# adamjorr/kbbq

Measured on AMD Instinct MI355X. Metric: recalibrated Gbases/sec, higher is better.
Workload: dtype u64

## Files before the change

### kbbq_amd/csrc/engine.hip

```cpp
#include <hip/hip_runtime.h>

#include <algorithm>
#include <cstdarg>
#include <cstdio>
#include <cstdlib>
#include <cstring>
#include <map>
#include <mutex>
#include <string>
#include <thread>
#include <vector>

#include "../../include/kbbq_engine.h"
#include "abi_internal.h"
#include "correct.h"
#include "correct_wave.h"
#include "device_common.h"
#include "host_model.h"

using namespace kbbq;

static thread_local char g_err[512] = "";
int kbbq_fail(int code, const char *fmt, ...) {
    va_list ap;
    va_start(ap, fmt);
    vsnprintf(g_err, sizeof g_err, fmt, ap);
    va_end(ap);
    return code;
}
#define fail kbbq_fail
#define HIP_TRY(expr)                                                                                  \
    do {                                                                                               \
        hipError_t _e = (expr);                                                                        \
        if (_e != hipSuccess)                                                                          \
            return fail(_e == hipErrorOutOfMemory ? KBBQ_ENOMEM : KBBQ_EIO, "%s: %s (%s:%d)", #expr,   \
                        hipGetErrorString(_e), __FILE__, __LINE__);                                    \
    } while (0)

#include "kernels.h"
#include "bucket.h"
#include "long_reads.h"


struct FilterHost {
    FilterSpec spec;
    uint64_t *d_table = nullptr;
    uint64_t *d_patterns = nullptr;
    unsigned long long *d_inserted = nullptr;
    uint64_t table_bytes() const { return spec.n_blocks * kEngineBlockBytes; }
    FiltDev dev() const {
        FiltDev f;
        f.table = reinterpret_cast<ulonglong2 *>(d_table);
        f.patterns = reinterpret_cast<const ulonglong2 *>(d_patterns);
        f.n_blocks = spec.n_blocks;
        const ModMagic mm = make_mod_magic(spec.n_blocks);
        f.mod_magic = mm.m64;
        f.mod_m32 = mm.m32;
        f.salt0 = spec.salt[0];
        f.salt1 = spec.salt[1];
        return f;
    }
};

struct ProfileSlot {
    std::string name;
    uint64_t launches = 0;
    double ms = 0;
};
struct PendingEvent {
    int slot;
    hipEvent_t a, b;
};

struct Options {
    bool no_overlap = false;
    bool no_fastpath = false;
    bool lane_walk = false;
    bool no_pass4_pipeline = false;
    int pass2_side = 2;
    bool tally_general = false;
    bool infer_subset = true;
    bool debug_bucket = false;
    int bucket = -1;
    uint64_t bucket_records = 0;
    uint64_t pass4_piece = 0;
    int scan_blocks = -1;
    int walk_blocks = -1;
    int infer_blocks = 0;
};

struct kbbq_engine {
    kbbq_params p;
    Options opt;
    KParams K;
    hipStream_t stream = nullptr;
    hipStream_t stream2 = nullptr;
    hipEvent_t ev_main = nullptr, ev_side[2] = {nullptr, nullptr};
    hipEvent_t ev_draw = nullptr, ev_ins[2] = {nullptr, nullptr};
    bool ins_pending[2] = {false, false};
    int draw_turn = 0;
    bool side_busy[2] = {false, false};
    bool pass3_shared = false;
    unsigned long long *d_totals = nullptr;
    int side_turn = 0;
    uint32_t *d_qpresent = nullptr;
    uint32_t qpresent[8] = {};
    bool qpresent_known = false;
    uint8_t *d_dq_qslot = nullptr;
    int dq_slots = 0;
    uint32_t *d_rg_present[2] = {nullptr, nullptr};
    hipStream_t cur = nullptr;
    unsigned long long *cur_cnt = nullptr;
    FilterHost filt[2];
    Xoshiro256 seed_state;
    uint64_t draw_threshold = 0;
    bool draw_always = false;
    bool thresholds_set = false;
    std::vector<int32_t> thresholds;
    unsigned long long *d_hist = nullptr;
    uint64_t hist_cycle_words = 0, hist_dinuc_words = 0;
    DqTables dq;
    bool dq_set = false;
    int16_t *d_dq_base = nullptr;
    int8_t *d_dq_cycle = nullptr;
    int8_t *d_dq_dinuc = nullptr;
    void *scratch[24] = {};
    size_t scratch_bytes[24] = {};
    unsigned long long *d_counters = nullptr;
    unsigned int *d_tickets = nullptr;
    struct StageSlot {
        char *dev = nullptr;
        size_t bytes = 0;
        hipEvent_t h2d = nullptr, done[2] = {nullptr, nullptr};
        hipEvent_t d2h = nullptr;
        bool busy[2] = {false, false};
        bool d2h_pending = false;
        uint32_t gen = 0;
    } slot[3];
    int slot_turn = 0, cur_slot = -1;
    bool cur_slot_side = false;
    bool cur_h2d_recorded = false;
    bool async_call = false;
    uint64_t last_ticket = 0;
    hipStream_t copy = nullptr;
    uint64_t stats[4] = {0, 0, 0, 0};
    std::vector<ProfileSlot> prof;
    std::vector<PendingEvent> pending;
    uint32_t *d_qcum = nullptr, *d_errthr = nullptr;
    uint32_t qcum_len = 0;
    struct Buckets {
        int mode[2] = {-1, -1};
        bool allocated = false;
        uint64_t capacity = 0;
        void *l1 = nullptr, *l2 = nullptr;
        uint32_t *l1_cnt = nullptr, *l2_cnt = nullptr, *tickets = nullptr;
        unsigned long long *direct = nullptr;
        bool pending[2] = {false, false};
        double pending_est[2] = {0, 0};
        double frac_trusted = 0.75;
        double frac_used = 0.75;
        uint64_t bases_since[2] = {0, 0}, inserted_at_flush[2] = {0, 0};
        uint64_t flushes[2] = {0, 0};
        hipStream_t stream[2] = {nullptr, nullptr};
        hipEvent_t ev_flush = nullptr;
        unsigned long long *h_inserted = nullptr;
        hipEvent_t ev_est = nullptr;
        bool est_pending = false, est_known = false;
        uint64_t est_bases = 0, est_prev = 0, cur_bases = 0;
    } bk;
    hipEvent_t ev_infer = nullptr, ev_take[2] = {nullptr, nullptr};
    bool take_pending[2] = {false, false};
    int take_turn = 0;
    size_t attr_lds_tally = 0, attr_lds_recal = 0;
    std::map<const void *, size_t> attr_lds_correct;
};

namespace {

int ensure_scratch(kbbq_engine *e, int idx, size_t bytes) {
    if (e->scratch_bytes[idx] >= bytes) return KBBQ_OK;
    if (e->scratch[idx]) {
        HIP_TRY(hipStreamSynchronize(e->stream));
        HIP_TRY(hipStreamSynchronize(e->stream2));
        HIP_TRY(hipFree(e->scratch[idx]));
        e->scratch[idx] = nullptr;
        e->scratch_bytes[idx] = 0;
    }
    const size_t want = bytes + bytes / 8 + 256;
    HIP_TRY(hipMalloc(&e->scratch[idx], want));
    e->scratch_bytes[idx] = want;
    return KBBQ_OK;
}

static void plan_tally_slots(TallyPlan &P, const uint32_t mask[8], int max_slots, int n_rg) {
    memset(P.qslot, 255, sizeof P.qslot);
    memset(P.qof, 0, sizeof P.qof);
    P.n_slots = 0;
    max_slots = std::max(1, std::min(max_slots, 255));
    int top = -1, distinct = 0;
    for (int q = 0; q < KBBQ_NQ; ++q)
        if ((mask[q >> 5] >> (q & 31)) & 1) { top = q; ++distinct; }
    if (top >= 0 && top + 1 <= max_slots && (n_rg <= 1 || 2 * distinct >= top + 1)) {
        for (int q = 0; q <= top; ++q) { P.qof[q] = (uint8_t)q; P.qslot[q] = (uint8_t)q; }
        P.n_slots = top + 1;
        P.identity = 1;
    } else {
        for (int q = 0; q < KBBQ_NQ && P.n_slots < max_slots; ++q)
            if ((mask[q >> 5] >> (q & 31)) & 1) { P.qof[P.n_slots] = (uint8_t)q; P.qslot[q] = (uint8_t)P.n_slots++; }
        P.identity = 0;
    }
    if (P.n_slots == 0) { P.n_slots = 1; P.qof[0] = 0; P.qslot[0] = 0; P.identity = 1; }
    P.rg_base = 0; P.n_rgs = 1; P.cbase = 0; P.direct_cycles = 0;
}

struct Timed {
    kbbq_engine *e;
    int slot = -1;
    hipEvent_t a = nullptr, b = nullptr;
    hipStream_t on = nullptr;
    Timed(kbbq_engine *e_, const char *name, hipStream_t stream = nullptr) : e(e_), on(stream ? stream : e_->stream) {
        if (!(e->p.flags & KBBQ_F_PROFILE)) return;
        for (size_t i = 0; i < e->prof.size(); ++i)
            if (e->prof[i].name == name) slot = (int)i;
        if (slot < 0) {
            ProfileSlot s;
            s.name = name;
            e->prof.push_back(s);
            slot = (int)e->prof.size() - 1;
        }
        hipEventCreate(&a);
        hipEventCreate(&b);
        hipEventRecord(a, on);
    }
    ~Timed() {
        if (slot < 0) return;
        hipEventRecord(b, on);
        PendingEvent pe = {slot, a, b};
        e->pending.push_back(pe);
    }
};

void drain_profile(kbbq_engine *e) {
    for (size_t i = 0; i < e->pending.size(); ++i) {
        PendingEvent &pe = e->pending[i];
        float ms = 0;
        if (hipEventSynchronize(pe.b) == hipSuccess && hipEventElapsedTime(&ms, pe.a, pe.b) == hipSuccess) {
            e->prof[pe.slot].ms += ms;
            e->prof[pe.slot].launches += 1;
        }
        hipEventDestroy(pe.a);
        hipEventDestroy(pe.b);
    }
    e->pending.clear();
}

__global__ void k_add_counters(const unsigned long long *side, const unsigned long long *offcase, unsigned long long *totals) {
// ... 359 lines not shown
        HIP_TRY(hipStreamWaitEvent(e->stream, b.ev_flush, 0));
    }
    if (w == 1 && !barrier) {
        bucket_poll_estimate(e);
        if (!b.est_pending && b.h_inserted) {
            HIP_TRY(hipMemcpyAsync(b.h_inserted, e->filt[1].d_inserted, 8, hipMemcpyDeviceToHost, e->stream));
            HIP_TRY(hipEventRecord(b.ev_est, e->stream));
            b.est_pending = true;
            b.est_bases = b.bases_since[1] + b.cur_bases;
            b.est_prev = b.inserted_at_flush[1];
            if (!b.est_known) {
                HIP_TRY(hipEventSynchronize(b.ev_est));
                bucket_poll_estimate(e);
                b.est_known = true;
            }
        }
    }
    {
        if (e->opt.debug_bucket) fprintf(stderr, "[bucket] flush %d of filter %d: estimate %.3g records over %llu bases (%.4f per base), barrier %d\n",
                           (int)b.flushes[w], w, b.pending_est[w], (unsigned long long)b.bases_since[w], w ? b.frac_trusted : 0.0, (int)barrier);
    }
    b.bases_since[w] = 0;
    b.pending[w] = false;
    b.pending_est[w] = 0;
    b.flushes[w] += 1;
    return KBBQ_OK;
}

int bucket_flush_all(kbbq_engine *e) {
    for (int w = 0; w < 2; ++w) {
        int rc = bucket_flush(e, w);
        if (rc) return rc;
    }
    return KBBQ_OK;
}

int bucket_reserve(kbbq_engine *e, int w, double est, uint64_t bases) {
    kbbq_engine::Buckets &b = e->bk;
    int rc = bucket_flush(e, 1 - w);
    if (rc) return rc;
    b.cur_bases = bases;
    if (b.pending[w] && b.pending_est[w] + est > 0.93 * (double)b.capacity) {
        if ((rc = bucket_flush(e, w, false))) return rc;
        if (w == 1) est = (est - 4096.0) / std::max(1e-9, b.frac_used) * b.frac_trusted + 4096.0;
    }
    b.cur_bases = 0;
    b.pending[w] = true;
    b.pending_est[w] += est;
    b.bases_since[w] += bases;
    return KBBQ_OK;
}

}


extern "C" {

const char *kbbq_last_error(void) { return g_err; }

int kbbq_engine_create(const kbbq_params *params, kbbq_engine **out) {
    if (!params || !out) return fail(KBBQ_EINVAL, "null argument");
    if (params->k < 1 || params->k > KBBQ_MAX_KMER) return fail(KBBQ_ERANGE, "k must be <= %d and > 0", KBBQ_MAX_KMER);
    if (params->n_rg < 1 || params->n_rg > 65535) return fail(KBBQ_EINVAL, "n_rg must be in 1..65535");
    if (params->max_read_len < 1 || params->max_read_len > KBBQ_MAX_READ_LEN)
        return fail(KBBQ_ERANGE, "max_read_len must be in 1..%d", KBBQ_MAX_READ_LEN);
    int ndev = 0;
    if (hipGetDeviceCount(&ndev) != hipSuccess || ndev == 0) return fail(KBBQ_ENODEV, "no HIP device visible");
    if (params->device < 0 || params->device >= ndev) return fail(KBBQ_ENODEV, "device %d of %d", params->device, ndev);
    DeviceGuard create_guard(params->device);
    HIP_TRY(create_guard.err);
    kbbq_engine *e = new kbbq_engine;
    e->p = *params;
    {
        Options &o = e->opt;
        auto env_set = [](const char *name) { const char *v = getenv(name); return v && *v; };
        auto env_int = [](const char *name, int dflt) { const char *v = getenv(name); return v && *v ? atoi(v) : dflt; };
        const int fl = params->flags;
        o.no_overlap = (fl & KBBQ_F_NO_OVERLAP) || env_set("KBBQ_NO_OVERLAP");
        o.no_fastpath = (fl & KBBQ_F_NO_FASTPATH) || env_set("KBBQ_NO_FASTPATH");
        o.lane_walk = (fl & KBBQ_F_LANE_WALK) || (getenv("KBBQ_CORRECT") && !strcmp(getenv("KBBQ_CORRECT"), "lane"));
        o.no_pass4_pipeline = (fl & KBBQ_F_NO_PASS4_PIPELINE) || env_set("KBBQ_NO_PASS4_PIPELINE");
        o.pass2_side = (fl & KBBQ_F_PASS2_INORDER) ? 0 : env_int("KBBQ_PASS2_SIDE", o.pass2_side);
        o.tally_general = env_set("KBBQ_TALLY_GENERAL");
        o.infer_subset = env_int("KBBQ_INFER_SUBSET", 1) != 0;
        o.debug_bucket = env_set("KBBQ_DEBUG_BUCKET");
        o.bucket = (fl & KBBQ_F_BUCKET_ON) ? 1 : (fl & KBBQ_F_BUCKET_OFF) ? 0 : env_set("KBBQ_BUCKET") ? (env_int("KBBQ_BUCKET", 0) != 0 ? 1 : 0) : -1;
        o.bucket_records = env_u64("KBBQ_BUCKET_RECORDS", 0);
        o.pass4_piece = env_u64("KBBQ_PASS4_PIECE", 0);
        o.scan_blocks = env_int("KBBQ_SCAN_BLOCKS", o.scan_blocks);
        o.walk_blocks = env_int("KBBQ_WALK_BLOCKS", o.walk_blocks);
        o.infer_blocks = env_int("KBBQ_INFER_BLOCKS", o.infer_blocks);
    }
    e->K.k = params->k;
    e->K.shift = 2u * (unsigned)(params->k - 1);
    e->K.mask = params->k < 32 ? ((1ULL << (2 * params->k)) - 1) : ~0ULL;
    e->K.nmask_bits = params->k < 32 ? ((1u << params->k) - 1) : 0xFFFFFFFFu;
    const double fprs[2] = {params->fpr_sampled, params->fpr_trusted};
    for (int w = 0; w < 2; ++w) {
        if (!make_filter_spec(params->approx_kmers, fprs[w], params->bloom_seed, e->filt[w].spec)) {
            delete e;
            return fail(KBBQ_EINVAL, "Error: Invalid bloom filter parameters. Adjust parameters and try again.");
        }
    }
    hipError_t he = hipStreamCreateWithFlags(&e->stream, hipStreamNonBlocking);
    if (he == hipSuccess) he = hipStreamCreateWithFlags(&e->stream2, hipStreamNonBlocking);
    if (he == hipSuccess) he = hipEventCreateWithFlags(&e->ev_main, hipEventDisableTiming);
    if (he == hipSuccess) he = hipEventCreateWithFlags(&e->ev_draw, hipEventDisableTiming);
    for (int t = 0; t < 2 && he == hipSuccess; ++t) he = hipEventCreateWithFlags(&e->ev_ins[t], hipEventDisableTiming);
    if (he == hipSuccess) he = hipEventCreateWithFlags(&e->ev_side[0], hipEventDisableTiming);
    if (he == hipSuccess) he = hipEventCreateWithFlags(&e->ev_side[1], hipEventDisableTiming);
    if (he == hipSuccess) he = hipStreamCreateWithFlags(&e->copy, hipStreamNonBlocking);
    if (he == hipSuccess) he = hipEventCreateWithFlags(&e->bk.ev_flush, hipEventDisableTiming);
    if (he == hipSuccess) he = hipEventCreateWithFlags(&e->bk.ev_est, hipEventDisableTiming);
    if (he == hipSuccess) he = hipEventCreateWithFlags(&e->ev_infer, hipEventDisableTiming);
    for (int t = 0; t < 2 && he == hipSuccess; ++t) he = hipEventCreateWithFlags(&e->ev_take[t], hipEventDisableTiming);
    if (he == hipSuccess) he = hipHostMalloc((void **)&e->bk.h_inserted, 64, hipHostMallocDefault);
    for (int i = 0; i < 3 && he == hipSuccess; ++i) {
        he = hipEventCreateWithFlags(&e->slot[i].h2d, hipEventDisableTiming);
        if (he == hipSuccess) he = hipEventCreateWithFlags(&e->slot[i].d2h, hipEventDisableTiming);
        for (int t = 0; t < 2 && he == hipSuccess; ++t) he = hipEventCreateWithFlags(&e->slot[i].done[t], hipEventDisableTiming);
    }
    e->cur = e->stream;
    if (he != hipSuccess) { kbbq_engine_destroy(e); return fail(KBBQ_EIO, "hipStreamCreate: %s", hipGetErrorString(he)); }
#define CREATE_TRY(expr)                                                                           \
    do {                                                                                           \
        hipError_t _e = (expr);                                                                    \
        if (_e != hipSuccess) {                                                                    \
            int code = _e == hipErrorOutOfMemory ? KBBQ_ENOMEM : KBBQ_EIO;                         \
            fail(code, "%s: %s", #expr, hipGetErrorString(_e));                                    \
            kbbq_engine_destroy(e);                                                                \
            return code;                                                                           \
        }                                                                                          \
    } while (0)
    CREATE_TRY(hipMalloc(&e->d_counters, 64));
    CREATE_TRY(hipMemset(e->d_counters, 0, 64));
    CREATE_TRY(hipMalloc(&e->d_tickets, 64));
    CREATE_TRY(hipMemset(e->d_tickets, 0, 64));
    CREATE_TRY(hipMalloc(&e->d_totals, 32));
    CREATE_TRY(hipMemset(e->d_totals, 0, 32));
    e->cur_cnt = e->d_counters;
    CREATE_TRY(hipMalloc(&e->d_dq_qslot, KBBQ_NQ));
    CREATE_TRY(hipMalloc(&e->d_qpresent, 32));
    for (int i = 0; i < 2; ++i) CREATE_TRY(hipMalloc(&e->d_rg_present[i], (((size_t)params->n_rg + 31) / 32) * 4 + 4));
    for (int w = 0; w < 2; ++w) {
        FilterHost &f = e->filt[w];
        CREATE_TRY(hipMalloc(&f.d_table, f.table_bytes()));
        CREATE_TRY(hipMalloc(&f.d_patterns, kNumPatterns * kEngineBlockBytes));
        CREATE_TRY(hipMalloc(&f.d_inserted, 8));
        std::vector<uint64_t> packed(kNumPatterns * 2);
        for (uint64_t i = 0; i < kNumPatterns; ++i) {
            if (!squeeze_block(&f.spec.patterns[i * 8], &packed[i * 2])) {
                kbbq_engine_destroy(e);
                return fail(KBBQ_ESTATE, "pattern %llu uses a bit outside the 128 the generator can reach", (unsigned long long)i);
            }
        }
        CREATE_TRY(hipMemcpy(f.d_patterns, packed.data(), kNumPatterns * kEngineBlockBytes, hipMemcpyHostToDevice));
    }
    e->hist_cycle_words = (uint64_t)params->n_rg * kNQ * 2 * params->max_read_len * 2;
    e->hist_dinuc_words = (uint64_t)params->n_rg * kNQ * 16 * 2;
    CREATE_TRY(hipMalloc(&e->d_hist, (e->hist_cycle_words + e->hist_dinuc_words) * 8));
    CREATE_TRY(hipMalloc(&e->d_dq_base, (size_t)params->n_rg * kNQ * 2));
    CREATE_TRY(hipMalloc(&e->d_dq_cycle, (size_t)params->n_rg * kNQ * 2 * params->max_read_len));
    CREATE_TRY(hipMalloc(&e->d_dq_dinuc, (size_t)params->n_rg * kNQ * 16));
    CREATE_TRY(hipMemcpyToSymbol(HIP_SYMBOL(c_jump), xoshiro_jump_table(), 64 * 4 * 8));
    e->seed_state.seed32(params->seed);
    e->draw_threshold = bernoulli_threshold(params->alpha, &e->draw_always);
// ... 29 lines not shown
        hipFree(e->filt[w].d_inserted);
    }
    hipFree(e->d_hist);
    hipFree(e->d_dq_base);
    hipFree(e->d_dq_cycle);
    hipFree(e->d_dq_dinuc);
    hipFree(e->d_counters);
    hipFree(e->d_tickets);
    hipFree(e->d_totals);
    hipFree(e->d_dq_qslot);
    hipFree(e->d_qpresent);
    hipFree(e->d_rg_present[0]);
    hipFree(e->d_rg_present[1]);
    hipFree(e->d_qcum);
    hipFree(e->d_errthr);
    hipFree(e->bk.l1); hipFree(e->bk.l2); hipFree(e->bk.l1_cnt); hipFree(e->bk.l2_cnt); hipFree(e->bk.tickets); hipFree(e->bk.direct);
    for (int i = 0; i < 24; ++i) hipFree(e->scratch[i]);
    if (e->stream2) { hipStreamSynchronize(e->stream2); hipStreamDestroy(e->stream2); }
    if (e->ev_main) hipEventDestroy(e->ev_main);
    if (e->ev_draw) hipEventDestroy(e->ev_draw);
    for (int t = 0; t < 2; ++t) if (e->ev_ins[t]) hipEventDestroy(e->ev_ins[t]);
    for (int i = 0; i < 2; ++i) if (e->ev_side[i]) hipEventDestroy(e->ev_side[i]);
    if (e->stream) hipStreamDestroy(e->stream);
    delete e;
}

int kbbq_engine_reset(kbbq_engine *e) {
    ENGINE_DEVICE(e);
    if (!e) return fail(KBBQ_EINVAL, "null engine");
    int rc0 = sync_engine(e);
    if (rc0) return rc0;
    for (int w = 0; w < 2; ++w) {
        HIP_TRY(hipMemsetAsync(e->filt[w].d_table, 0, e->filt[w].table_bytes(), e->stream));
        HIP_TRY(hipMemsetAsync(e->filt[w].d_inserted, 0, 8, e->stream));
    }
    HIP_TRY(hipMemsetAsync(e->d_hist, 0, (e->hist_cycle_words + e->hist_dinuc_words) * 8, e->stream));
    HIP_TRY(hipMemsetAsync(e->d_counters, 0, 64, e->stream));
    HIP_TRY(hipMemsetAsync(e->d_totals, 0, 16, e->stream));
    HIP_TRY(hipMemsetAsync(e->d_qpresent, 0, 32, e->stream));
    memset(e->qpresent, 0, sizeof e->qpresent);
    e->qpresent_known = false;
    if (e->bk.allocated) {
        HIP_TRY(hipMemsetAsync(e->bk.l1_cnt, 0, kL1CntBytes, e->stream));
        HIP_TRY(hipMemsetAsync(e->bk.l2_cnt, 0, kL2CntBytes, e->stream));
        HIP_TRY(hipMemsetAsync(e->bk.direct, 0, 8, e->stream));
    }
    e->bk.est_pending = false;
    e->bk.est_known = false;
    e->bk.frac_trusted = 0.75;
    e->bk.stream[0] = e->bk.stream[1] = nullptr;
    for (int w = 0; w < 2; ++w) { e->bk.pending[w] = false; e->bk.pending_est[w] = 0; e->bk.bases_since[w] = 0; e->bk.inserted_at_flush[w] = 0; e->bk.flushes[w] = 0; }
    e->thresholds_set = false;
    e->dq_set = false;
    memset(e->stats, 0, sizeof e->stats);
    return sync_engine(e);
}

int kbbq_engine_sync(kbbq_engine *e) {
    ENGINE_DEVICE(e);
    { int frc = bucket_flush_all(e); if (frc) return frc; }
    if (!e) return fail(KBBQ_EINVAL, "null engine");
    return sync_engine(e);
}

void *kbbq_engine_stream(kbbq_engine *e) { return e ? (void *)e->stream : nullptr; }

int kbbq_engine_dims(kbbq_engine *e, uint64_t *n_rg, uint64_t *n_cycle) {
    if (!e) return fail(KBBQ_EINVAL, "null engine");
    if (n_rg) *n_rg = (uint64_t)e->p.n_rg;
    if (n_cycle) *n_cycle = (uint64_t)e->p.max_read_len;
    return KBBQ_OK;
}

int kbbq_engine_tune(kbbq_engine *e, const char *name, uint64_t value) {
    if (!e || !name) return fail(KBBQ_EINVAL, "null argument");
    if (!strcmp(name, "bucket_records")) {
        if (e->bk.allocated) return fail(KBBQ_ESTATE, "the record buffers are allocated already");
        e->opt.bucket_records = value;
    } else if (!strcmp(name, "pass4_piece")) {
        e->opt.pass4_piece = value;
    } else if (!strcmp(name, "scan_blocks") || !strcmp(name, "walk_blocks") || !strcmp(name, "infer_blocks")) {
        if (value > 17) return fail(KBBQ_EINVAL, "%s: 0 (as many as fit) to 16 workgroups per CU, 17 = default", name);
        (name[0] == 's' ? e->opt.scan_blocks : name[0] == 'w' ? e->opt.walk_blocks : e->opt.infer_blocks) = value == 17 ? (name[0] == 'i' ? 0 : -1) : (int)value;
    } else if (!strcmp(name, "infer_subset")) {
        e->opt.infer_subset = value != 0;
    } else if (!strcmp(name, "pass2_side")) {
        ENGINE_DEVICE(e);
        { int frc = bucket_flush_all(e); if (frc) return frc; }
        int rc = sync_engine(e);
        if (rc) return rc;
        if (value > 2) return fail(KBBQ_EINVAL, "pass2_side: 0, 1 or 2");
        e->opt.pass2_side = (int)value;
        e->bk.stream[0] = e->bk.stream[1] = nullptr;
    } else if (!strcmp(name, "no_overlap")) {
        ENGINE_DEVICE(e);
        { int frc = bucket_flush_all(e); if (frc) return frc; }
        int rc = sync_engine(e);
        if (rc) return rc;
        e->opt.no_overlap = value != 0;
        e->bk.stream[0] = e->bk.stream[1] = nullptr;
    } else {
        return fail(KBBQ_EINVAL, "unknown knob '%s'", name);
    }
    return KBBQ_OK;
}

int kbbq_filter_info_get(kbbq_engine *e, int which, kbbq_filter_info *out) {
    ENGINE_DEVICE(e);
    { int frc = bucket_flush_all(e); if (frc) return frc; }
    if (!e || !out || which < 0 || which > 1) return fail(KBBQ_EINVAL, "bad argument");
    const FilterSpec &s = e->filt[which].spec;
    memset(out, 0, sizeof *out);
    out->bits = s.bits;
    out->bits_unblocked = s.bits_unblocked;
    out->n_blocks = s.n_blocks;
    out->table_bytes = e->filt[which].table_bytes();
    out->random_seed = s.random_seed;
    out->n_hash = s.n_hash;
    out->n_salt = s.n_salt;
    for (uint32_t i = 0; i < s.n_salt; ++i) out->salt[i] = s.salt[i];
    int rc = sync_engine(e);
    if (rc) return rc;
    HIP_TRY(hipMemcpy(&out->inserted, e->filt[which].d_inserted, 8, hipMemcpyDeviceToHost));
    return KBBQ_OK;
}

void *kbbq_filter_device_table(kbbq_engine *e, int which) {
    if (!e || which < 0 || which > 1) return nullptr;
    DeviceGuard guard(e->p.device);
    if (guard.err != hipSuccess || bucket_flush_all(e) != KBBQ_OK) return nullptr;
    return e->filt[which].d_table;
}
void *kbbq_filter_device_counter(kbbq_engine *e, int which) { return e && which >= 0 && which < 2 ? e->filt[which].d_inserted : nullptr; }

int kbbq_filter_download(kbbq_engine *e, int which, uint64_t *host_words, uint64_t n_words) {
    ENGINE_DEVICE(e);
    { int frc = bucket_flush_all(e); if (frc) return frc; }
    if (!e || !host_words || which < 0 || which > 1) return fail(KBBQ_EINVAL, "bad argument");
    const uint64_t n_blocks = e->filt[which].spec.n_blocks;
    if (n_words != n_blocks * 8) return fail(KBBQ_EINVAL, "filter has %llu words", (unsigned long long)n_blocks * 8);
    int rc = sync_engine(e);
    if (rc) return rc;
    const uint64_t chunk = 1 << 20;
    std::vector<uint64_t> packed(chunk * 2);
    for (uint64_t b0 = 0; b0 < n_blocks; b0 += chunk) {
        const uint64_t nb = std::min(chunk, n_blocks - b0);
        HIP_TRY(hipMemcpy(packed.data(), e->filt[which].d_table + b0 * 2, nb * kEngineBlockBytes, hipMemcpyDeviceToHost));
        for (uint64_t b = 0; b < nb; ++b) expand_block(&packed[b * 2], host_words + (b0 + b) * 8);
    }
    return KBBQ_OK;
}

int kbbq_filter_patterns_download(kbbq_engine *e, int which, uint64_t *host_words) {
    ENGINE_DEVICE(e);
    if (!e || !host_words || which < 0 || which > 1) return fail(KBBQ_EINVAL, "bad argument");
    std::vector<uint64_t> packed(kNumPatterns * 2);
    HIP_TRY(hipMemcpy(packed.data(), e->filt[which].d_patterns, kNumPatterns * kEngineBlockBytes, hipMemcpyDeviceToHost));
    for (uint64_t i = 0; i < kNumPatterns; ++i) expand_block(&packed[i * 2], host_words + i * 8);
    return KBBQ_OK;
}

int kbbq_filter_or_from(kbbq_engine *e, int which, const void *src_device, uint64_t word_offset, uint64_t n_words) {
    ENGINE_DEVICE(e);
    { int frc = bucket_flush_all(e); if (frc) return frc; }
    if (!e || !src_device || which < 0 || which > 1) return fail(KBBQ_EINVAL, "bad argument");
    const uint64_t total = e->filt[which].spec.n_blocks * 2;
// ... 773 lines not shown
        raised = lds;
    }
    Timed t(e, "k_correct", e->cur);
    const int blocks = (int)std::min<uint64_t>((R.n_reads + BLOCK - 1) / BLOCK, 256 * 8);
    hipLaunchKernelGGL((k_correct<MAXL, BLOCK>), dim3(blocks), dim3(BLOCK), lds, e->cur, R, e->K, e->filt[1].dev(), list,
                       n_list, tmask, tw, err_bits, patch, e->cur_cnt, 0, (uint32_t *)nullptr);
    HIP_TRY(hipGetLastError());
    return KBBQ_OK;
}

template <int NB, int NN>
static int launch_correct_wave(kbbq_engine *e, ReadsDev R, const uint32_t *list, const uint64_t *tmask, int tw,
                               uint32_t *err_bits, uint32_t *patch) {
    unsigned int *ticket = e->d_tickets + 3 + (e->cur_cnt != e->d_counters ? 1 : 0);
    HIP_TRY(hipMemsetAsync(ticket, 0, 4, e->cur));
    Timed t(e, "k_correct_wave", e->cur);
    const int blocks = wave_grid(R.n_reads, e->pass3_shared ? shared_cap(e, e->opt.walk_blocks, 2, NB <= 5 ? 160 : 512, !R.offsets) : 0);
    hipLaunchKernelGGL((k_correct_wave<NB, NN>), dim3(blocks), dim3(256), 0, e->cur, R, e->K, e->filt[1].dev(), list,
                       (const unsigned long long *)e->cur_cnt, tmask, tw, err_bits, patch, e->cur_cnt, ticket);
    HIP_TRY(hipGetLastError());
    return KBBQ_OK;
}
extern "C" {

static int build_read_index(kbbq_engine *e, const ReadsDev &R, int slot, hipStream_t stream, const uint32_t **index) {
    *index = nullptr;
    if (!R.offsets || !R.n_reads) return KBBQ_OK;
    const size_t entries = R.n_bases / READ_INDEX_STEP + 2;
    int rc = ensure_scratch(e, slot, entries * 4);
    if (rc) return rc;
    hipLaunchKernelGGL(k_read_index, dim3((unsigned)((R.n_reads + 255) / 256)), dim3(256), 0, stream, R.offsets, R.n_reads, (uint32_t *)e->scratch[slot]);
    HIP_TRY(hipGetLastError());
    *index = (const uint32_t *)e->scratch[slot];
    return KBBQ_OK;
}

static int run_tally(kbbq_engine *e, const ReadsDev &R, const uint32_t *err_bits, const uint32_t *patch, int max_len,
                     hipStream_t stream = nullptr) {
    if (!stream) stream = e->cur;
    HistDev H;
    H.cycle = e->d_hist;
    H.dinuc = e->d_hist + e->hist_cycle_words;
    H.n_rg = e->p.n_rg;
    H.n_cycle = e->p.max_read_len;
    const int n_rg = R.rg ? e->p.n_rg : 1;
    const int ccap = std::min(((max_len + 31) / 32) * 32, 192);
    if (!e->qpresent_known) {
        hipLaunchKernelGGL(k_qpresence, dim3(1024), dim3(256), 0, stream, R.qual, R.n_bases, e->d_qpresent);
        HIP_TRY(hipGetLastError());
        HIP_TRY(hipMemcpyAsync(e->qpresent, e->d_qpresent, 32, hipMemcpyDeviceToHost, stream));
        HIP_TRY(hipStreamSynchronize(stream));
    }
    const int n_windows = (max_len + ccap - 1) / ccap;
    const bool direct_cycles = n_windows > kTallyMaxWindows;
    const size_t per_slot = (direct_cycles ? 0 : (size_t)8 * ccap) + 128;
    TallyPlan P;
    plan_tally_slots(P, e->qpresent, (int)((152 * 1024 - 512) / per_slot), n_rg);
    P.direct_cycles = direct_cycles ? 1 : 0;
    const size_t per_rg = (size_t)P.n_slots * per_slot;
    const size_t budget = (size_t)n_rg * per_rg <= 70 * 1024 ? 70 * 1024 : 140 * 1024;
    const int per_launch = (int)std::max<size_t>(1, std::min<size_t>((size_t)n_rg, budget / per_rg));
    const size_t lds = (size_t)per_launch * per_rg + 4 + 256 + 4;
    if (lds > e->attr_lds_tally) {
        HIP_TRY(hipFuncSetAttribute((const void *)k_tally, hipFuncAttributeMaxDynamicSharedMemorySize, (int)lds));
        HIP_TRY(hipFuncSetAttribute((const void *)k_tally_uniform<true>, hipFuncAttributeMaxDynamicSharedMemorySize, (int)lds));
        HIP_TRY(hipFuncSetAttribute((const void *)k_tally_uniform<false>, hipFuncAttributeMaxDynamicSharedMemorySize, (int)lds));
        e->attr_lds_tally = lds;
    }
    const uint64_t groups = (R.n_bases + 15) / 16;
    const int blocks = (int)std::min<uint64_t>((groups + 1023) / 1024, lds <= 76 * 1024 ? 512 : 256);
    const int vec_ok = ((uintptr_t)R.qual & 15) == 0;
    const uint32_t *read_index;
    int rc = build_read_index(e, R, stream == e->stream2 ? 15 : 14, stream, &read_index);
    if (rc) return rc;
    const uint32_t *present = nullptr;
    if (n_rg > per_launch) {
        uint32_t *pr = e->d_rg_present[stream == e->stream2 ? 1 : 0];
        HIP_TRY(hipMemsetAsync(pr, 0, (((size_t)e->p.n_rg + 31) / 32) * 4, stream));
        hipLaunchKernelGGL(k_rg_presence, dim3((unsigned)((R.n_reads + 255) / 256)), dim3(256), 0, stream, R.rg, R.n_reads, (uint32_t)e->p.n_rg, pr);
        present = pr;
    }
    if (!e->opt.tally_general && !R.offsets && n_rg == 1 && n_windows == 1 && R.read_len >= 16 && (int)R.read_len <= ccap && R.n_bases < (1ULL << 32) && vec_ok &&
        e->p.n_rg == 1) {
        const unsigned long long inv_len = ~0ULL / R.read_len + 1;
        Timed t(e, "k_tally", stream);
        if (P.identity) hipLaunchKernelGGL(k_tally_uniform<false>, dim3(blocks), dim3(1024), lds, stream, R, H, err_bits, patch, ccap, 6, inv_len, P);
        else hipLaunchKernelGGL(k_tally_uniform<true>, dim3(blocks), dim3(1024), lds, stream, R, H, err_bits, patch, ccap, 6, inv_len, P);
        HIP_TRY(hipGetLastError());
        return KBBQ_OK;
    }
    Timed t(e, "k_tally", stream);
    for (int g = 0; g < n_rg; g += per_launch)
        for (int w = 0; w < (direct_cycles ? 1 : n_windows); ++w) {
            P.rg_base = g;
            P.n_rgs = std::min(per_launch, n_rg - g);
            P.cbase = w * ccap;
            hipLaunchKernelGGL(k_tally, dim3(blocks), dim3(1024), lds, stream, R, H, err_bits, patch, ccap, 6, vec_ok, P, present, read_index);
        }
    HIP_TRY(hipGetLastError());
    return KBBQ_OK;
}

int kbbq_errors_batch(kbbq_engine *e, const kbbq_reads *reads, uint64_t *errors_out) {
    ENGINE_DEVICE(e);
    { int frc = bucket_flush_all(e); if (frc) return frc; }
    if (!e || !reads) return fail(KBBQ_EINVAL, "null argument");
    const bool own_err = !(errors_out && reads->on_device);
    const bool overlap = own_err && !(errors_out && !reads->on_device) && !e->opt.no_overlap;
    int side = 0, rc;
    if (overlap) {
        side = e->side_turn;
        e->side_turn ^= 1;
        if (e->side_busy[side]) HIP_TRY(hipStreamWaitEvent(e->stream, e->ev_side[side], 0));
    } else {
        if ((rc = sync_engine(e))) return rc;
    }
    e->pass3_shared = overlap;
    HostBatchDone host_done(e, reads);
    ReadsDev R; int max_len;
    if ((rc = device_view(e, reads, &R, &max_len))) return rc;
    const bool long_reads = max_len > kStagedMax;
    const int NW = max_len <= 192 ? 3 : max_len <= 320 ? 5 : !long_reads ? 8 : 8 * ((std::max(1, max_len - e->p.k + 1) + 511) / 512);
    const int s_tmask = side ? 10 : 3, s_dirty = side ? 11 : 4, s_list = side ? 12 : 5, s_err = side ? 8 : 6, s_patch = side ? 9 : 7;
    if ((rc = ensure_scratch(e, s_tmask, R.n_reads * NW * 8))) return rc;
    if ((rc = ensure_scratch(e, s_dirty, R.n_reads))) return rc;
    if ((rc = ensure_scratch(e, s_list, R.n_reads * 4))) return rc;
    if ((rc = ensure_scratch(e, s_patch, R.n_reads * 4))) return rc;
    uint32_t *d_err;
    if (own_err) {
        if ((rc = ensure_scratch(e, s_err, (R.n_bases / 64 + 2) * 8))) return rc;
        d_err = (uint32_t *)e->scratch[s_err];
    } else {
        d_err = (uint32_t *)errors_out;
    }
    e->cur = e->stream;
    e->cur_cnt = e->d_counters + 4 * side;
    struct Restore { kbbq_engine *e; ~Restore() { e->cur = e->stream; e->cur_cnt = e->d_counters; } } restore = {e};
    HIP_TRY(hipMemsetAsync(d_err, 0, (R.n_bases / 64 + 1) * 8, e->cur));
    HIP_TRY(hipMemsetAsync(e->scratch[s_patch], 0, R.n_reads * 4, e->cur));
    HIP_TRY(hipMemsetAsync(e->cur_cnt, 0, 16, e->cur));
    uint64_t *tmask = (uint64_t *)e->scratch[s_tmask];
    uint8_t *dirty = (uint8_t *)e->scratch[s_dirty];
    uint32_t *list = (uint32_t *)e->scratch[s_list];
    uint32_t *patch = (uint32_t *)e->scratch[s_patch];
    const bool no_fast = e->opt.no_fastpath;
    if (long_reads) {
        Timed t(e, "k_scan_trusted_long", e->cur);
        hipLaunchKernelGGL(k_scan_trusted_long, dim3(wave_grid(R.n_reads)), dim3(256), 0, e->cur, R, e->K, e->filt[1].dev(), tmask, NW, dirty);
        HIP_TRY(hipGetLastError());
    } else if ((rc = dispatch_nw<LaunchScan>(max_len, e, R, tmask, dirty, d_err, (!no_fast && e->p.k >= 3) ? 1 : 0, max_len))) return rc;
    {
        Timed t(e, "k_compact", e->cur);
        hipLaunchKernelGGL(k_compact, dim3((unsigned)((R.n_reads + 1023) / 1024)), dim3(1024), 0, e->cur, dirty, R.n_reads, list, e->cur_cnt,
                           long_reads ? 0 : 1);
        HIP_TRY(hipGetLastError());
    }
    if (overlap) {
        HIP_TRY(hipEventRecord(e->ev_main, e->stream));
        HIP_TRY(hipStreamWaitEvent(e->stream2, e->ev_main, 0));
        e->cur = e->stream2;
        e->cur_slot_side = true;
    }
    const bool lane_form = e->opt.lane_walk;
    if (long_reads) {
        rc = launch_correct<0, 64>(e, R, list, e->cur_cnt, tmask, NW, d_err, patch, max_len, side);
    } else if (lane_form || e->p.k < 3) {
// ... 470 lines not shown
```

### kbbq_amd/csrc/kernels.h

```cpp
#pragma once
#include <hip/hip_runtime.h>

#include "../../include/kbbq_engine.h"
#include "correct.h"
#include "correct_wave.h"
#include "device_common.h"

using namespace kbbq;


constexpr int DRAWS_PER_LANE = 4096;

__constant__ uint64_t c_jump[64][4];

__device__ __forceinline__ uint64_t xo_next(uint64_t (&s)[4]) {
    uint64_t x = s[1] * 5;
    x = (x << 7) | (x >> 57);
    x *= 9;
    const uint64_t t = s[1] << 17;
    s[2] ^= s[0];
    s[3] ^= s[1];
    s[1] ^= s[2];
    s[0] ^= s[3];
    s[2] ^= t;
// ... 984 lines not shown
                const int c = (slot % cstep) * 16 + slot / cstep;
                if (c < H.n_cycle) {
                    atomicAdd(&H.cycle[cyc_index(H, 0, q, sec, c) + 1], (unsigned long long)cnt);
                    if (cne) atomicAdd(&H.cycle[cyc_index(H, 0, q, sec, c)], (unsigned long long)cne);
                }
            }
        }
        for (int w = threadIdx.x; w < ns * 16; w += blockDim.x) {
            const uint32_t v = t_di[w], ve = t_die[w];
            const uint64_t cell = (uint64_t)(MAP ? (int)P.qof[w >> 4] : (w >> 4)) * 16 + (w & 15);
            if (v) { t_di[w] = 0; atomicAdd(&H.dinuc[cell * 2 + 1], (unsigned long long)v); }
            if (ve) { t_die[w] = 0; atomicAdd(&H.dinuc[cell * 2], (unsigned long long)ve); }
        }
    };
    const uint64_t n_groups = (R.n_bases + 15) / 16;
    const uint64_t stride = (uint64_t)gridDim.x * blockDim.x;
    const uint64_t iters = (n_groups + stride - 1) / stride;
    const uint64_t flush_every = max((uint64_t)1, (uint64_t)40000 / ((uint64_t)16384 / (uint64_t)L + 2));
    for (uint64_t it = 0; it < iters; ++it) {
        const uint64_t g0 = (it * stride + (uint64_t)blockIdx.x * blockDim.x + threadIdx.x) * 16;
        if (g0 + 16 <= R.n_bases) {
            const uint32_t r = (uint32_t)__umul64hi((unsigned long long)g0, inv_len);
            const int c0 = (int)(g0 - (uint64_t)r * (uint64_t)L);
            const int bpos = L - c0 < 16 ? L - c0 : 16;
            const uint4 qv4 = *reinterpret_cast<const uint4 *>(R.qual + g0);
            uint8_t qv[16];
            memcpy(qv, &qv4, 16);
            const uint32_t bw = (uint32_t)(R.bases[g0 >> 5] >> ((g0 & 31) * 2));
            const uint32_t nw = (uint32_t)(R.nmask[g0 >> 6] >> (g0 & 63)) & 0xFFFFu;
            const uint32_t ew = (err_bits[g0 >> 5] >> (g0 & 31)) & 0xFFFFu;
            int prev_b = 0, prev_n = 1;
            if (g0 > 0) {
                const uint64_t gp = g0 - 1;
                prev_b = (int)((R.bases[gp >> 5] >> ((gp & 31) * 2)) & 3);
                prev_n = (int)((R.nmask[gp >> 6] >> (gp & 63)) & 1);
            }
            const bool two = bpos < 16;
            const bool mine1 = !R.rg || R.rg[r] == 0, mine2 = !two || !R.rg || R.rg[r + 1] == 0;
            const int sec1 = R.flags ? (R.flags[r] & 1) : 0;
            const int sec2 = two && R.flags ? (R.flags[r + 1] & 1) : 0;
            const uint32_t pt1 = patch ? patch[r] : 0u, pt2 = two && patch ? patch[r + 1] : 0u;
            const int pp1 = (pt1 >> 31) ? patch_at(pt1) : -2, pp2 = (pt2 >> 31) ? patch_at(pt2) : -2;
            if (pp1 >= 0 && pp1 == c0 - 1) { prev_b = (int)(pt1 & 3); prev_n = 0; }
#pragma unroll
            for (int i = 0; i < 16; ++i) {
                const bool in2 = i >= bpos;
                const int cyc = c0 + i - (in2 ? L : 0);
                int b = (int)((bw >> (2 * i)) & 3), nn = (int)((nw >> i) & 1);
                if (cyc == (in2 ? pp2 : pp1)) { b = (int)((in2 ? pt2 : pt1) & 3); nn = 0; }
                const int q = qv[i];
                if (in2 ? mine2 : mine1)
                    count(in2 ? sec2 : sec1, q, cyc, (int)((ew >> i) & 1u), cyc >= 1 && q >= minscore && !(nn | prev_n), (prev_b << 2) | b);
                prev_b = b;
                prev_n = nn;
            }
        } else if (g0 < R.n_bases) {
            for (uint64_t g = g0; g < R.n_bases; ++g) {
                const uint64_t r = g / (uint64_t)L;
                const int cyc = (int)(g - r * (uint64_t)L);
                const uint32_t pt = patch ? patch[r] : 0u;
                const int pp = (pt >> 31) ? patch_at(pt) : -2;
                auto base_at = [&](uint64_t x, int cx, int &bb, int &nb) {
                    bb = (int)((R.bases[x >> 5] >> ((x & 31) * 2)) & 3);
                    nb = (int)((R.nmask[x >> 6] >> (x & 63)) & 1);
                    if (cx == pp) { bb = (int)(pt & 3); nb = 0; }
                };
                int b, nn, pb = 0, pn = 1;
                base_at(g, cyc, b, nn);
                if (cyc >= 1) base_at(g - 1, cyc - 1, pb, pn);
                const int q = R.qual[g];
                const int er = (int)((err_bits[g >> 5] >> (g & 31)) & 1u);
                if (!R.rg || R.rg[r] == 0)
                    count(R.flags ? (R.flags[r] & 1) : 0, q, cyc, er, cyc >= 1 && q >= minscore && !(nn | pn), (pb << 2) | b);
            }
        }
        if ((it + 1) % flush_every == 0 || it + 1 == iters) {
            __syncthreads();
            flush();
            __syncthreads();
        }
    }
}

__global__ void __launch_bounds__(256) k_qpresence(const uint8_t *qual, uint64_t n_bases, uint32_t *qpresent) {
    __shared__ uint32_t qseen[8];
    if (threadIdx.x < 8) qseen[threadIdx.x] = 0;
    __syncthreads();
    for (uint64_t i = (uint64_t)blockIdx.x * blockDim.x + threadIdx.x; i < n_bases; i += (uint64_t)gridDim.x * blockDim.x)
        qseen_note(qseen, qual[i]);
    __syncthreads();
    if (threadIdx.x < 8 && qseen[threadIdx.x]) atomicOr(&qpresent[threadIdx.x], qseen[threadIdx.x]);
}

struct DqDev {
    const int16_t *base;
    const int8_t *cycle;
    const int8_t *dinuc;
    const uint8_t *qslot;
    int n_rg, n_cycle, n_slots;
};

__global__ void __launch_bounds__(1024) k_recalibrate(ReadsDev R, DqDev D, uint8_t *out, int minqual, int vec_ok, int lds_rgs,
                                                       const uint32_t *read_index, uint64_t base0, uint64_t base1) {
    extern __shared__ uint8_t l_tab[];
    uint8_t *l_qslot = l_tab;
    const int ns = D.n_slots;
    const int cyc_cells = ns * 2 * D.n_cycle, di_bytes = ns * 16, base_bytes = KBBQ_NQ * 2;
    const int cyc_bytes = 2 * cyc_cells;
    const int per_rg = (cyc_bytes + di_bytes + base_bytes + 3) & ~3;
    uint8_t *l_rg = l_tab + 256;
    if (threadIdx.x < 256) l_qslot[threadIdx.x] = D.qslot[threadIdx.x];
    __syncthreads();
    for (int i = threadIdx.x; i < lds_rgs * KBBQ_NQ; i += blockDim.x) {
        const int rg = i / KBBQ_NQ, q = i % KBBQ_NQ;
        reinterpret_cast<int16_t *>(l_rg + (size_t)rg * per_rg + cyc_bytes + di_bytes)[q] = D.base[rg * KBBQ_NQ + q];
        const int sl = l_qslot[q];
        if (sl != 255) {
            int16_t *tc = reinterpret_cast<int16_t *>(l_rg + (size_t)rg * per_rg) + sl * 2 * D.n_cycle;
            const int8_t *src = D.cycle + ((size_t)rg * KBBQ_NQ + q) * 2 * D.n_cycle;
            for (int c = 0; c < 2 * D.n_cycle; ++c) tc[c] = (int16_t)(D.base[rg * KBBQ_NQ + q] + src[c]);
            for (int x = 0; x < 16; ++x) l_rg[(size_t)rg * per_rg + cyc_bytes + sl * 16 + x] = (uint8_t)D.dinuc[((size_t)rg * KBBQ_NQ + q) * 16 + x];
        }
    }
    __syncthreads();
    for (uint64_t g0 = base0 + ((uint64_t)blockIdx.x * blockDim.x + threadIdx.x) * 16; g0 < base1;
         g0 += (uint64_t)gridDim.x * blockDim.x * 16) {
    uint64_t r, start, end;
    if (R.offsets) {
        find_read(R, read_index, g0, r, start, end);
    } else {
        r = g0 / R.read_len;
        start = r * R.read_len;
        end = start + R.read_len;
    }
    const int n = (int)min((uint64_t)16, R.n_bases - g0);
    uint8_t qv[16];
    if (n == 16 && vec_ok) {
        const uint4 v = *reinterpret_cast<const uint4 *>(R.qual + g0);
        memcpy(qv, &v, 16);
    } else {
        for (int i = 0; i < 16; ++i) qv[i] = i < n ? R.qual[g0 + i] : 0;
    }
    const uint32_t bw = (uint32_t)(R.bases[g0 >> 5] >> ((g0 & 31) * 2));
    const uint32_t nw = (uint32_t)(R.nmask[g0 >> 6] >> (g0 & 63)) & 0xFFFFu;
    int prev_b = 0, prev_n = 1;
    if (g0 > 0) {
        const uint64_t gp = g0 - 1;
        prev_b = (int)((R.bases[gp >> 5] >> ((gp & 31) * 2)) & 3);
        prev_n = (int)((R.nmask[gp >> 6] >> (gp & 63)) & 1);
    }
    int rg = R.rg ? (int)R.rg[r] : 0;
    int second = R.flags ? (R.flags[r] & 1) : 0;
    uint8_t res[16];
    const int bpos = end - g0 < 16 ? (int)(end - g0) : 16;
    int rg2 = rg, second2 = second;
    uint64_t end2 = end;
    if (bpos < 16 && r + 1 < R.n_reads) {
        rg2 = R.rg ? (int)R.rg[r + 1] : 0;
        second2 = R.flags ? (R.flags[r + 1] & 1) : 0;
        end2 = R.offsets ? R.offsets[r + 2] : end + R.read_len;
    }
    const int c0 = (int)(g0 - start);
    const bool plain = n == 16 && rg < lds_rgs && rg2 < lds_rgs && (bpos == 16 || (r + 1 < R.n_reads && end2 >= g0 + 16)) &&
                       c0 + bpos <= D.n_cycle && 16 - bpos <= D.n_cycle;
    if (plain) {
        const int16_t *ta = reinterpret_cast<const int16_t *>(l_rg + rg * per_rg) + second * D.n_cycle + c0;
// ... 154 lines not shown
```

Measured before the change: 23.16.

## Add column-layout tally kernel with rotated LDS bins and replicated dinuc counters

Adds k_tally_cols, the new default for the uniform single-read-group tally path. Each wave covers whole reads split into 16-base segments, with lane-rotated indexing so LDS atomics spread across banks. Cycle counts go into per-column bins and dinucleotide counts into replicated bins with packed 16-bit totals and errors, folded and flushed periodically. Loads for the next iteration are fetched while the current one is processed. It aims to cut LDS atomic contention and per-base decode overhead in the tally, but adds an alternate slow path, register pressure and extra folding syncs.

Result: faster. 23.66 (median of 6 runs) (+2.1%).

```diff
diff --git a/kbbq_amd/csrc/engine.hip b/kbbq_amd/csrc/engine.hip
--- a/kbbq_amd/csrc/engine.hip
+++ b/kbbq_amd/csrc/engine.hip
@@ -79,6 +79,7 @@
     bool no_pass4_pipeline = false;
     int pass2_side = 2;
     bool tally_general = false;
+    int tally_kernel = 0;
     bool infer_subset = true;
     bool debug_bucket = false;
     int bucket = -1;
@@ -171,7 +172,7 @@
     hipEvent_t ev_infer = nullptr, ev_take[2] = {nullptr, nullptr};
     bool take_pending[2] = {false, false};
     int take_turn = 0;
-    size_t attr_lds_tally = 0, attr_lds_recal = 0;
+    size_t attr_lds_tally = 0, attr_lds_recal = 0, attr_lds_tally_cols = 0;
     std::map<const void *, size_t> attr_lds_correct;
 };
 
@@ -697,6 +698,7 @@
         o.no_pass4_pipeline = (fl & KBBQ_F_NO_PASS4_PIPELINE) || env_set("KBBQ_NO_PASS4_PIPELINE");
         o.pass2_side = (fl & KBBQ_F_PASS2_INORDER) ? 0 : env_int("KBBQ_PASS2_SIDE", o.pass2_side);
         o.tally_general = env_set("KBBQ_TALLY_GENERAL");
+        o.tally_kernel = env_int("KBBQ_TALLY_KERNEL", 0);
         o.infer_subset = env_int("KBBQ_INFER_SUBSET", 1) != 0;
         o.debug_bucket = env_set("KBBQ_DEBUG_BUCKET");
         o.bucket = (fl & KBBQ_F_BUCKET_ON) ? 1 : (fl & KBBQ_F_BUCKET_OFF) ? 0 : env_set("KBBQ_BUCKET") ? (env_int("KBBQ_BUCKET", 0) != 0 ? 1 : 0) : -1;
@@ -892,6 +894,9 @@
     } else if (!strcmp(name, "scan_blocks") || !strcmp(name, "walk_blocks") || !strcmp(name, "infer_blocks")) {
         if (value > 17) return fail(KBBQ_EINVAL, "%s: 0 (as many as fit) to 16 workgroups per CU, 17 = default", name);
         (name[0] == 's' ? e->opt.scan_blocks : name[0] == 'w' ? e->opt.walk_blocks : e->opt.infer_blocks) = value == 17 ? (name[0] == 'i' ? 0 : -1) : (int)value;
+    } else if (!strcmp(name, "tally_kernel")) {
+        if (value > 1) return fail(KBBQ_EINVAL, "tally_kernel: 0 (k_tally_cols) or 1 (k_tally_uniform)");
+        e->opt.tally_kernel = (int)value;
     } else if (!strcmp(name, "infer_subset")) {
         e->opt.infer_subset = value != 0;
     } else if (!strcmp(name, "pass2_side")) {
@@ -1831,6 +1836,35 @@
     }
     if (!e->opt.tally_general && !R.offsets && n_rg == 1 && n_windows == 1 && R.read_len >= 16 && (int)R.read_len <= ccap && R.n_bases < (1ULL << 32) && vec_ok &&
         e->p.n_rg == 1) {
+        if (e->opt.tally_kernel == 0) {
+            TallyColsShape T;
+            T.S = ((int)R.read_len + 15) / 16;
+            T.rpw = 64 / T.S;
+            T.nr = P.n_slots + (P.identity ? 0 : 1);
+            T.wr = ((T.rpw * T.S + 15 * T.S) + 31) / 32 * 32;
+            T.reps = 32;
+            auto cols_lds = [&](int reps) { return (size_t)4 * (2 * T.nr * T.wr + T.nr * 16 * reps + T.nr * 32) + 256; };
+            while (T.reps > 1 && cols_lds(T.reps) > 160 * 1024) T.reps /= 2;
+            const size_t clds = cols_lds(T.reps);
+            if (T.nr <= 127 && clds <= 160 * 1024) {
+                T.di_every = std::max(1, 65535 / (16 * (64 / T.reps) * 16));
+                T.cyc_every = std::max(1, 65535 / (16 * std::min(16, T.rpw)));
+                if (clds > e->attr_lds_tally_cols) {
+                    HIP_TRY(hipFuncSetAttribute((const void *)k_tally_cols<false>, hipFuncAttributeMaxDynamicSharedMemorySize, (int)clds));
+                    HIP_TRY(hipFuncSetAttribute((const void *)k_tally_cols<true>, hipFuncAttributeMaxDynamicSharedMemorySize, (int)clds));
+                    e->attr_lds_tally_cols = clds;
+                }
+                int cus = 0;
+                HIP_TRY(hipDeviceGetAttribute(&cus, hipDeviceAttributeMultiprocessorCount, e->p.device));
+                const uint64_t tiles = (R.n_reads + 16 * (uint64_t)T.rpw - 1) / (16 * (uint64_t)T.rpw);
+                const int cblocks = (int)std::max<uint64_t>(1, std::min<uint64_t>(tiles, (uint64_t)std::max(cus, 1)));
+                Timed t(e, "k_tally", stream);
+                if (P.identity) hipLaunchKernelGGL(k_tally_cols<false>, dim3(cblocks), dim3(1024), clds, stream, R, H, err_bits, patch, 6, P, T);
+                else hipLaunchKernelGGL(k_tally_cols<true>, dim3(cblocks), dim3(1024), clds, stream, R, H, err_bits, patch, 6, P, T);
+                HIP_TRY(hipGetLastError());
+                return KBBQ_OK;
+            }
+        }
         const unsigned long long inv_len = ~0ULL / R.read_len + 1;
         Timed t(e, "k_tally", stream);
         if (P.identity) hipLaunchKernelGGL(k_tally_uniform<false>, dim3(blocks), dim3(1024), lds, stream, R, H, err_bits, patch, ccap, 6, inv_len, P);
diff --git a/kbbq_amd/csrc/kernels.h b/kbbq_amd/csrc/kernels.h
--- a/kbbq_amd/csrc/kernels.h
+++ b/kbbq_amd/csrc/kernels.h
@@ -1090,6 +1090,236 @@
     }
 }
 
+struct TallyColsShape {
+    int S, rpw;
+    int nr, wr;
+    int reps;
+    int di_every;
+    int cyc_every;
+};
+
+__device__ __forceinline__ uint32_t rot16(uint32_t v, int r) { return ((v | (v << 16)) >> r) & 0xFFFFu; }
+__device__ __forceinline__ uint32_t bytes_of_bits(uint32_t m4) {
+    return __builtin_amdgcn_perm(0u, 0u, ((m4 * 0x00204081u) & 0x01010101u) + 0x0C0C0C0Cu);
+}
+__device__ __forceinline__ void lds_add_at(uint32_t *base, uint32_t byte_off, uint32_t v) {
+    atomicAdd(reinterpret_cast<uint32_t *>(reinterpret_cast<char *>(base) + byte_off), v);
+}
+
+template <bool MAP>
+__global__ void __launch_bounds__(1024) k_tally_cols(ReadsDev R, HistDev H, const uint32_t *err_bits, const uint32_t *patch,
+                                                     int minscore, TallyPlan P, TallyColsShape T) {
+    extern __shared__ uint32_t lds[];
+    if (R.n_reads == 0) return;
+    const int L = (int)R.read_len, S = T.S, rpw = T.rpw, nr = T.nr, wr = T.wr, reps = T.reps;
+    uint32_t *t_cyc = lds;
+    uint32_t *t_rep = lds + 2 * nr * wr;
+    uint32_t *t_di = t_rep + nr * 16 * reps;
+    uint8_t *l_qslot = reinterpret_cast<uint8_t *>(t_di + nr * 32);
+    const int words = 2 * nr * wr + nr * 16 * reps + nr * 32;
+    for (int i = threadIdx.x; i < words; i += blockDim.x) lds[i] = 0;
+    if (MAP && threadIdx.x < 256) l_qslot[threadIdx.x] = P.qslot[threadIdx.x];
+    __syncthreads();
+
+    const int lane = threadIdx.x & 63;
+    const int rs = lane / S, seg = lane - rs * S, rr = rs & 15;
+    const bool lane_on = rs < rpw;
+    const int nb = min(16, L - 16 * seg);
+    const uint32_t seg_ok = ((1u << nb) - 1u) & (seg == 0 ? 0xFFFEu : 0xFFFFu);
+    const uint32_t col0 = (uint32_t)lane * 4u, colS = (uint32_t)S * 4u, rowb = (uint32_t)wr * 4u;
+    const uint32_t rep4 = (uint32_t)(lane & (reps - 1)) * 4u;
+    const int rep_shift = __builtin_ctz((unsigned)reps) + 2;
+    const uint32_t n = (uint32_t)R.n_bases;
+    const uint32_t nbw = (n + 15) / 16 - 1, nnw = (n + 31) / 32 - 1;
+    const uint32_t *bases32 = reinterpret_cast<const uint32_t *>(R.bases);
+    const uint32_t *nmask32 = reinterpret_cast<const uint32_t *>(R.nmask);
+    const uint32_t n_reads = (uint32_t)R.n_reads;
+    const uint32_t waves = gridDim.x * (blockDim.x >> 6);
+    const uint32_t wave0 = blockIdx.x * (blockDim.x >> 6) + (threadIdx.x >> 6);
+    const uint32_t per_it = waves * (uint32_t)rpw;
+    const uint32_t iters = (n_reads + per_it - 1) / per_it;
+
+    struct Raw { uint4 q; uint32_t b0, b1, bp, n0, n1, np, e0, e1, pt, g0; int sec, act; };
+    auto fetch = [&](uint32_t it) {
+        Raw w;
+        const uint32_t r1 = (it * waves + wave0) * (uint32_t)rpw + (uint32_t)rs;
+        w.act = lane_on && it < iters && r1 < n_reads;
+        const uint32_t r = w.act ? r1 : 0u;
+        if (w.act && R.rg && R.rg[r] != 0) w.act = 0;
+        const uint32_t g0 = r * (uint32_t)L + 16u * (uint32_t)seg;
+        w.g0 = g0;
+        const uint32_t qa = min(g0, n - 16u);
+        __builtin_memcpy(&w.q, R.qual + qa, 16);
+        const uint32_t bi = g0 >> 4, ni = g0 >> 5;
+        w.b0 = bases32[bi];
+        w.b1 = bases32[min(bi + 1u, nbw)];
+        w.bp = bases32[bi ? bi - 1u : 0u];
+        w.n0 = nmask32[ni];
+        w.n1 = nmask32[min(ni + 1u, nnw)];
+        w.np = nmask32[ni ? ni - 1u : 0u];
+        w.e0 = err_bits[ni];
+        w.e1 = err_bits[min(ni + 1u, nnw)];
+        w.sec = R.flags ? (R.flags[r] & 1) : 0;
+        w.pt = patch ? patch[r] : 0u;
+        return w;
+    };
+
+    auto fold_reps = [&]() {
+        for (int k = threadIdx.x; k < nr * 16; k += blockDim.x) {
+            uint32_t tot = 0, er = 0;
+            for (int p = 0; p < reps; ++p) {
+                const uint32_t v = t_rep[k * reps + p];
+                t_rep[k * reps + p] = 0;
+                tot += v & 0xFFFFu;
+                er += v >> 16;
+            }
+            t_di[2 * k] += tot;
+            t_di[2 * k + 1] += er;
+        }
+    };
+    auto flush_cycles = [&]() {
+        for (int w = threadIdx.x; w < 2 * nr * wr; w += blockDim.x) {
+            const uint32_t v = t_cyc[w];
+            if (!v) continue;
+            t_cyc[w] = 0;
+            const int srow = w / wr, col = w - srow * wr;
+            const int c = 16 * (col % S) + ((col / S) & 15);
+            const int row = srow % nr, sec = srow / nr;
+            if (c >= L || c >= H.n_cycle || (MAP && row == 0)) continue;
+            const int q = MAP ? (int)P.qof[row - 1] : row;
+            atomicAdd(&H.cycle[cyc_index(H, 0, q, sec, c) + 1], (unsigned long long)(v & 0xFFFFu));
+            if (v >> 16) atomicAdd(&H.cycle[cyc_index(H, 0, q, sec, c)], (unsigned long long)(v >> 16));
+        }
+    };
+    auto flush_dinuc = [&]() {
+        for (int k = threadIdx.x; k < nr * 16; k += blockDim.x) {
+            const uint32_t tot = t_di[2 * k], er = t_di[2 * k + 1];
+            const int row = k >> 4;
+            if (!tot || (MAP && row == 0)) continue;
+            const int q = MAP ? (int)P.qof[row - 1] : row;
+            if (q < minscore) continue;
+            const uint64_t cell = (uint64_t)q * 16 + (k & 15);
+            atomicAdd(&H.dinuc[cell * 2 + 1], (unsigned long long)tot);
+            if (er) atomicAdd(&H.dinuc[cell * 2], (unsigned long long)er);
+        }
+    };
+
+    auto step = [&](uint32_t it, const Raw &w) {
+        if (w.act) {
+            const uint32_t g0 = w.g0, sb = g0 & 15u, sn = g0 & 31u;
+            uint32_t B = __builtin_amdgcn_alignbit(w.b1, w.b0, 2u * sb);
+            uint32_t N = __builtin_amdgcn_alignbit(w.n1, w.n0, sn) & 0xFFFFu;
+            const uint32_t E = __builtin_amdgcn_alignbit(w.e1, w.e0, sn) & 0xFFFFu;
+            uint32_t pb = sb ? (w.b0 >> (2u * sb - 2u)) & 3u : w.bp >> 30;
+            uint32_t pn = sn ? (w.n0 >> (sn - 1u)) & 1u : w.np >> 31;
+            if (w.pt >> 31) {
+                const int x = patch_at(w.pt) - 16 * seg;
+                if ((unsigned)x < 16u) {
+                    B = (B & ~(3u << (2 * x))) | ((w.pt & 3u) << (2 * x));
+                    N &= ~(1u << x);
+                } else if (x == -1) {
+                    pb = w.pt & 3u;
+                    pn = 0;
+                }
+            }
+            const uint32_t P2 = (B << 2) | pb;
+            const uint32_t ok = ~(N | (N << 1) | pn) & seg_ok;
+            const uint32_t Br = __builtin_amdgcn_alignbit(B, B, 2u * rr), Pr = __builtin_amdgcn_alignbit(P2, P2, 2u * rr);
+            const uint32_t okr = rot16(ok, rr), Er = rot16(E, rr) << 16;
+            uint32_t q4[4] = {w.q.x, w.q.y, w.q.z, w.q.w};
+            {
+                const int t = (rr + (int)(g0 - min(g0, n - 16u))) & 15, dw = t >> 2, sh = (t & 3) * 8;
+                uint32_t a0 = q4[0], a1 = q4[1], a2 = q4[2], a3 = q4[3];
+                if (dw & 2) { uint32_t x0 = a0, x1 = a1; a0 = a2; a1 = a3; a2 = x0; a3 = x1; }
+                if (dw & 1) { uint32_t x0 = a0; a0 = a1; a1 = a2; a2 = a3; a3 = x0; }
+                q4[0] = __builtin_amdgcn_alignbit(a1, a0, sh);
+                q4[1] = __builtin_amdgcn_alignbit(a2, a1, sh);
+                q4[2] = __builtin_amdgcn_alignbit(a3, a2, sh);
+                q4[3] = __builtin_amdgcn_alignbit(a0, a3, sh);
+            }
+            uint32_t row4[4];
+            bool slow = false;
+            if (MAP) {
+#pragma unroll
+                for (int k = 0; k < 4; ++k) {
+                    uint32_t v = 0;
+#pragma unroll
+                    for (int b = 0; b < 4; ++b) {
+                        const uint32_t sl = l_qslot[(q4[k] >> (8 * b)) & 0xFFu];
+                        slow = slow || sl == 255u;
+                        v |= ((sl + 1u) & 0xFFu) << (8 * b);
+                    }
+                    row4[k] = v;
+                }
+            } else {
+                const uint32_t K = (uint32_t)(128 - P.n_slots) * 0x01010101u;
+                uint32_t hi = 0;
+#pragma unroll
+                for (int k = 0; k < 4; ++k) { row4[k] = q4[k]; hi |= (q4[k] + K) | q4[k]; }
+                slow = (hi & 0x80808080u) != 0;
+            }
+            const uint32_t soff = (uint32_t)(w.sec * nr) * 0x01010101u;
+            if (!slow) {
+#pragma unroll
+                for (int k = 0; k < 4; ++k) {
+                    const uint32_t qc = row4[k] + soff;
+                    const uint32_t qd = row4[k] & bytes_of_bits((okr >> (4 * k)) & 15u);
+#pragma unroll
+                    for (int b = 0; b < 4; ++b) {
+                        const int i = 4 * k + b;
+                        const uint32_t val = 1u | (((Er >> i) & 0x10000u));
+                        lds_add_at(t_cyc, __umul24((qc >> (8 * b)) & 0xFFu, rowb) + col0 + (uint32_t)i * colS, val);
+                        const uint32_t key = ((((qd >> (8 * b)) & 0xFFu) * 4u + ((Pr >> (2 * i)) & 3u)) * 4u) + ((Br >> (2 * i)) & 3u);
+                        lds_add_at(t_rep, (key << rep_shift) + rep4, val);
+                    }
+                }
+            } else {
+#pragma unroll
+                for (int i = 0; i < 16; ++i) {
+                    const int x = (i + rr) & 15;
+                    const uint32_t q = (q4[i >> 2] >> (8 * (i & 3))) & 0xFFu;
+                    const uint32_t row = (row4[i >> 2] >> (8 * (i & 3))) & 0xFFu;
+                    const bool has_row = MAP ? row != 0 : q < (uint32_t)P.n_slots;
+                    const uint32_t er = (Er >> (16 + i)) & 1u, val = 1u | (er << 16);
+                    const bool di = (okr >> i) & 1u;
+                    const uint32_t d = (((Pr >> (2 * i)) & 3u) << 2) | ((Br >> (2 * i)) & 3u);
+                    if (has_row) {
+                        lds_add_at(t_cyc, (row + (uint32_t)(w.sec * nr)) * rowb + col0 + (uint32_t)i * colS, val);
+                        lds_add_at(t_rep, ((((di ? row : 0u) * 16u) + d) << rep_shift) + rep4, val);
+                    } else if (x < nb) {
+                        const int c = 16 * seg + x;
+                        atomicAdd(&H.cycle[cyc_index(H, 0, (int)q, w.sec, c) + 1], 1ULL);
+                        if (er) atomicAdd(&H.cycle[cyc_index(H, 0, (int)q, w.sec, c)], 1ULL);
+                        if (di && (int)q >= minscore) {
+                            atomicAdd(&H.dinuc[((uint64_t)q * 16 + d) * 2 + 1], 1ULL);
+                            if (er) atomicAdd(&H.dinuc[((uint64_t)q * 16 + d) * 2], 1ULL);
+                        }
+                    }
+                }
+            }
+        }
+        const bool last = it + 1 == iters;
+        const bool fold = last || (it + 1) % (uint32_t)T.di_every == 0;
+        const bool fcyc = last || (it + 1) % (uint32_t)T.cyc_every == 0;
+        if (fold || fcyc) {
+            __syncthreads();
+            if (fold) fold_reps();
+            if (fcyc) flush_cycles();
+            __syncthreads();
+        }
+    };
+    Raw a = fetch(0);
+    for (uint32_t it = 0; it < iters; it += 2) {
+        const Raw b = fetch(it + 1);
+        step(it, a);
+        if (it + 1 >= iters) break;
+        a = fetch(it + 2);
+        step(it + 1, b);
+    }
+    if (iters == 0) return;
+    flush_dinuc();
+}
+
 __global__ void __launch_bounds__(256) k_qpresence(const uint8_t *qual, uint64_t n_bases, uint32_t *qpresent) {
     __shared__ uint32_t qseen[8];
     if (threadIdx.x < 8) qseen[threadIdx.x] = 0;
```
